# spdes/chirpgp

Hardware: AMD Instinct MI355X
Metric: filter+smoother trial-steps/s (batch x T / wall) (higher is better)
Workload: dtype f64; 1 GPU; C2: discrete EKF+EKS (demos/ekfs_mle.py model); d=4, T=10000, batch_per_gpu=1000, global_batch=1000, parallelism=trials sharded x1

## Files before the change

### chirpgp_amd/csrc/cgp_mfma4.hpp

```cpp
#pragma once
#include "cgp_coop4.hpp"

namespace cgp {


CGP_DEV double mfma4(double a, double b, double c) { return __builtin_amdgcn_mfma_f64_4x4x4f64(a, b, c, 0, 0, 0); }

constexpr int kCheckedChunks = 16;

struct Ekf4MfmaConst {
    double M0, M1, M2, M3, rho, ang;
    double Hr, Xi, Sig;
    double kc, ks, kj, kk;
    double SigHq, c0;
    double kcr, ksr, kja;
    double angm;
    double pa, pb, pA0, pB0, m1, m2;
    CGP_DEV void fold() { kcr = kc * rho; ksr = ks * rho; kja = kj * ang; angm = (kc != 0.0 || ks != 0.0) ? ang : 0.0; }
    CGP_DEV void fold_e1(int r, int q) {
        fold();
        angm = q == 0 ? ang : (q == 1 ? -ang : 0.0);
        pa = q < 2 ? rho : 0.0;
        pb = q == 0 ? -rho : (q == 1 ? rho : 0.0);
        pA0 = q == 2 ? M0 : (q == 3 ? M3 : 0.0);
        pB0 = q == 2 ? M1 : (q == 3 ? M2 : 0.0);
        m1 = r == q ? 1.0 : 0.0;
        m2 = r == (q ^ 1) ? 1.0 : 0.0;
    }
    template <bool E1> CGP_DEV void load(const HarmonicLCD<1>& model, const FilterIO& io, int64_t trial, int r, int q) {
        M0 = model.M[0]; M1 = model.M[1]; M2 = model.M[2]; M3 = model.M[3];
        rho = model.rho;
        ang = (model.dt * kTwoPi) * model.fs;
        Hr = io.H[trial * io.H_stride + r];
        Xi = io.Xi[trial * io.Xi_stride];
        Sig = lane_sigma_entry(model, r, q);
        const double mq = model.q;
        SigHq = (q == 1) ? mq : 0.0;
        c0 = mq + Xi;
        kc = ((q == 0 && r == 0) || (q == 1 && r == 1)) ? 1.0 : 0.0;
        ks = (q == 0 && r == 1) ? -1.0 : ((q == 1 && r == 0) ? 1.0 : 0.0);
        kj = (r == 2 && q == 0) ? -1.0 : ((r == 2 && q == 1) ? 1.0 : 0.0);
        kk = (q == 2) ? (r == 2 ? M0 : (r == 3 ? M1 : 0.0)) : ((q == 3) ? (r == 2 ? M2 : (r == 3 ? M3 : 0.0)) : 0.0);
        if constexpr (E1) fold_e1(r, q);
        else fold();
    }
};
struct Ekf4State {
    double P, ur, uq;
    CGP_DEV double u2() const { return dpp_f64<kQuadBcast2>(uq); }
    CGP_DEV double u2_replicated() const { return row_bcast_f64<2>(uq); }
    template <bool E1> CGP_DEV void load(const FilterIO& io, int64_t trial, int r, int q) {
        const double* __restrict__ m0p = io.m0 + trial * io.m0_stride;
        ur = E1 ? 0.0 : m0p[r]; uq = m0p[q];
        P = coop4_load_sym_entry(io.P0 + trial * io.P0_stride, r, q);
    }
};

template <int E1 = 0, bool GAPS = false>
CGP_DEV void ekf4_mfma_finish_j(const Ekf4MfmaConst& K, double y, double A, double B2, double kjd, Ekf4State& x, double& S, double& innov) {
    double J0T, f_r, f_q;
    if constexpr (E1 != 0) {
        f_q = fma(A, x.uq, B2 * dpp_f64<kQuadSwap1>(x.uq));
        J0T = fma(K.m1, A, K.m2 * B2);
        f_r = 0.0;
    } else {
        J0T = A;
        f_r = mfma4(J0T, x.ur, 0.0); f_q = mfma4(x.ur, J0T, 0.0);
    }
    const double RJT = fma(kjd, dpp_f64<kQuadSwap1>(f_q), J0T);
    double Pp, PHr, PHq;
    if constexpr (E1 != 0) {
        auto bcast1 = [](double v) { if constexpr (E1 == 2) return row_bcast_f64<1>(v); else return dpp_f64<kQuadBcast1>(v); };
        const double Q = mfma4(x.P, RJT, 0.0);
        const double Pa = bcast1(Q);
        PHq = mfma4(Pa, RJT, K.SigHq);
        Pp = mfma4(RJT, Q, K.Sig);
        PHr = bcast1(Pp);
        if constexpr (E1 == 1) {
            const double a = dpp_f64<kQuadBcast1>(RJT);
            S = mfma4(a, Pa, K.c0);
        } else {
            S = bcast1(PHq) + K.Xi;
        }
        innov = y - bcast1(f_q);
    } else {
        const double Q = mfma4(x.P, RJT, 0.0);
        Pp = mfma4(RJT, Q, K.Sig);
        PHr = mfma4(Pp, K.Hr, 0.0);
        PHq = mfma4(K.Hr, Pp, 0.0);
        S = mfma4(K.Hr, PHr, K.Xi);
        innov = y - mfma4(K.Hr, f_r, 0.0);
    }
    double rS = rcp_nr1(S), dy = innov;
    if constexpr (GAPS) {
        const bool gap = is_missing(y);
        rS = gap ? 0.0 : rS;
        dy = gap ? 0.0 : innov;
    }
    x.P = fma(-(PHr * rS), PHq, Pp);
    const double g = rS * dy;
    if constexpr (E1 == 0) x.ur = fma(PHr, g, f_r);
    x.uq = fma(PHq, g, f_q);
}
template <int E1 = 0, bool GAPS = false>
CGP_DEV void ekf4_mfma_finish(const Ekf4MfmaConst& K, double y, double c1, double s1, double dsp, Ekf4State& x, double& S, double& innov) {
    if constexpr (E1 != 0) {
        ekf4_mfma_finish_j<E1, GAPS>(K, y, fma(K.pa, c1, K.pA0), fma(K.pb, s1, K.pB0), K.kja * dsp, x, S, innov);
    } else {
        const double J0T = fma(K.kcr, c1, fma(K.ksr, s1, K.kk));
        ekf4_mfma_finish_j<E1, GAPS>(K, y, J0T, 0.0, K.kja * dsp, x, S, innov);
    }
}

template <int E1 = 0, bool GAPS = false>
CGP_DEV void ekf4_mfma_step_wide(const Ekf4MfmaConst& K, const WideRegs& W, double y, Ekf4State& x, double& S, double& innov, bool& bad) {
    double sp, dsp, s1, c1;
    bool ok1, ok2;
    softplus_pair_any(W, x.u2(), sp, dsp, ok1);
    fast_sincos_spec(W, K.ang * sp, s1, c1, ok2);
    bad = bad || !(ok1 && ok2);
    ekf4_mfma_finish<E1, GAPS>(K, y, c1, s1, dsp, x, S, innov);
}

template <int E1 = 0, bool GAPS = false>
CGP_DEV void ekf4_mfma_step_checked(const Ekf4MfmaConst& K, double y, Ekf4State& x, double& S, double& innov) {
    double sp, dsp, s1, c1;
    softplus_pair_uniform(x.u2(), sp, dsp);
    fast_sincos_uniform(K.ang * sp, s1, c1);
    ekf4_mfma_finish<E1, GAPS>(K, y, c1, s1, dsp, x, S, innov);
}

struct Ekf4Anchor {
    double th, A, B;
    template <int E1 = 0>
    CGP_DEV void set(const Ekf4MfmaConst& K, double sp, double c1, double s1) {
        th = K.angm * sp;
        if constexpr (E1 != 0) {
            A = fma(K.pa, c1, K.pA0);
            B = fma(K.pb, s1, K.pB0);
        } else {
            A = fma(K.kcr, c1, fma(K.ksr, s1, K.kk));
            B = fma(K.ksr, c1, -(K.kcr * s1));
        }
    }
};

template <int E1 = 0>
CGP_DEV void ekf4_anchor(const Ekf4MfmaConst& K, double u2, Ekf4Anchor& a) {
    double sp, dsp, s1, c1;
    softplus_pair_uniform(u2, sp, dsp);
    fast_sincos_uniform(K.ang * sp, s1, c1);
    a.template set<E1>(K, sp, c1, s1);
}

constexpr unsigned kIncrementBound = 0x3F780000u;
constexpr int kRegCommon = 0, kRegHigh = 1, kRegLow = 2, kRegAny = 3, kRegMid = 4;
struct Ekf4Verdict {
    unsigned u = 0u, umin = 0xFFFFFFFFu, d = 0u;
    int di = 0;
    bool any_bad = false;
    unsigned uabs = 0u;
    template <int REG = kRegCommon> CGP_DEV bool state_in_regime() const {
        if constexpr (REG == kRegAny) return !any_bad;
        if constexpr (REG == kRegMid) return uabs < 0x40000000u;
        if constexpr (REG == kRegLow) return umin >= 0xBFF80000u && u <= 0xC085DFFFu;
        constexpr unsigned lo = REG == kRegHigh ? 0x40140000u : 0x3FF80000u;
        return u <= 0x4085DFFFu && umin >= lo;
    }
    template <int REG = kRegCommon> CGP_DEV unsigned code() const {
        const bool state = __builtin_amdgcn_ballot_w64(!state_in_regime<REG>()) != 0;
        const bool jump = __builtin_amdgcn_ballot_w64((d & 0x7FFFFFFFu) >= kIncrementBound || ((unsigned)di & 0x7FFFFFFFu) >= kIncrementBound) != 0;
        return (state ? 1u : 0u) | (jump ? 2u : 0u);
    }
    template <int REG = kRegCommon> CGP_DEV unsigned long long uncommon() const {
        return __builtin_amdgcn_ballot_w64(!state_in_regime<REG>()) |
               __builtin_amdgcn_ballot_w64((d & 0x7FFFFFFFu) >= kIncrementBound || ((unsigned)di & 0x7FFFFFFFu) >= kIncrementBound);
    }
};
template <int E1, int REG = kRegCommon>
CGP_DEV void ekf4_mfma_step_spec1(const Ekf4MfmaConst& K, const SpecRegs& R, const SpecRegsHigh& RH, double y, Ekf4State& x, Ekf4Anchor& a,
                                  double& S, double& innov, Ekf4Verdict& verdict, const SpecRegsMid* RM = nullptr, const WideRegs* RW = nullptr) {
    const double u2 = (E1 == 2) ? x.u2_replicated() : x.u2();
    constexpr bool HIGH = REG == kRegHigh, LOW = REG == kRegLow, ANY = REG == kRegAny, MID = REG == kRegMid;
    double d, jfac;
    if constexpr (MID) {
        double ga, hj;
        softplus_mid_polys(*RM, u2, ga, hj);
        d = ga + fma(0.5 * K.angm, u2, -a.th);
        jfac = fma(u2, hj, 0.5 * K.kja);
    } else if constexpr (ANY) {
        double sp, dspf; bool ok;
        if (RW) softplus_pair_any(*RW, u2, sp, dspf, ok);
        else softplus_pair_any(u2, sp, dspf, ok);
        verdict.any_bad = verdict.any_bad || !ok;
        d = fma(K.angm, sp, -a.th);
        jfac = K.kja * dspf;
    } else {
        const double t = HIGH ? exp_neg_high(R, RH, u2) : exp_neg_lean1(R, LOW ? -u2 : u2);
        const double lin = LOW ? -a.th : fma(K.angm, u2, -a.th);
        double qa, dsp;
        if constexpr (HIGH) softplus_tail_high(RH, t, qa, dsp);
        else softplus_tail_lean(R, t, qa, dsp);
        d = fma(qa, t, lin);
        jfac = HIGH ? dsp : LOW ? (K.kja * t) * dsp : K.kja * dsp;
    }
    const double d2 = d * d;
    const double tau = d * fma(d2, R.c4, 0.5);
    const double sn = d * fma(d2, R.s3, 1.0);
    const double A1 = fma(tau, a.B, a.A);
    const double B = fma(-sn, A1, a.B);
    const double A = fma(tau, B, A1);
    const unsigned hx = (unsigned)__double2hiint(u2), hd = (unsigned)__double2hiint(d);
    if constexpr (MID) {
        const unsigned ha = hx & 0x7FFFFFFFu;
        verdict.uabs = verdict.uabs > ha ? verdict.uabs : ha;
    } else if constexpr (!ANY) {
        verdict.u = verdict.u > hx ? verdict.u : hx;
        verdict.umin = verdict.umin < hx ? verdict.umin : hx;
    }
    verdict.d = verdict.d > hd ? verdict.d : hd;
    verdict.di = verdict.di > (int)hd ? verdict.di : (int)hd;
    a.th += d; a.A = A; a.B = B;
    ekf4_mfma_finish_j<E1>(K, y, A, B, jfac, x, S, innov);
}

constexpr int kEkf4Unroll = 4;

#ifdef CGP_EKF4_KERNELS
template <bool E1>
CGP_DEV void ekf4_mfma_trial(const FilterIO& io, const ModelArgs& ma) {
    const int lane = threadIdx.x;
    const int r = lane >> 4, q = lane & 3;
    const FilterSpan span = filter_span(io, blockIdx.x);
    using Seg = SegRecord<4>;
    const int64_t trial = span.trial;

    HarmonicLCD<1> model;
    model.setup(ma.params + trial * ma.param_stride, ma.dt, ma.model_id);
    Ekf4MfmaConst K;
    K.template load<E1>(model, io, trial, r, q);
    Ekf4State x;
    x.template load<E1>(io, trial, r, q);
    const double* __restrict__ ys = io.record(trial);
    Tile4FilterOut out;
    out.init(io, trial, lane);
    const unsigned p_off = out.offP, m_off = out.offm;
    const bool nll_final = (io.flags & CGP_NLL_FINAL_ONLY) != 0;
    double* __restrict__ nll = (io.nll && !nll_final) ? io.nll + trial * io.T : nullptr;
    const bool want_nll = io.nll != nullptr;

    SpecRegs R;
    R.init(K.angm);
    SpecRegsHigh RH;
    RH.init(K.angm, K.kja);
    constexpr int kParkStride = 2;
    __shared__ double2 park[64 * kParkStride];
    __shared__ double ybuf[64 + 16];
    double cum = 0.0;
    int checked_left = 0, spec_off = 0, jump_streak = 0, spec_score = -4;
    unsigned n_high = 0, n_common = 0, n_redo = 0, n_checked = 0, n_high_left = 0, n_wide = 0, n_low = 0, n_mid = 0;
    Ekf4Anchor anchor_live;
    int anchor_age = -1;
    const int64_t Te = span.t_end;
    double ynext = (span.t_begin + lane < Te) ? ys[span.t_begin + lane] : 0.0;
    for (int64_t t0 = span.t_begin; t0 < Te; t0 += 64) {
        wave_lds_fence();
        const bool burn = t0 < span.t_out;
        const OobWindow Pw = out.P_window(burn), mw = out.m_window(burn);
        if (span.state && span.seg > 0 && t0 == span.t_out) {
            Seg::put_mean(span.state, Seg::kJunction, lane < 4, lane, x.uq);
            Seg::put_cov(span.state, Seg::kJunction, ((lane >> 2) & 3) == 0, r, q, x.P);
        }
        double ychunk = ynext;
        asm volatile("" : "+v"(ychunk));
        ynext = (t0 + 64 + lane < Te) ? ys[t0 + 64 + lane] : 0.0;
        const int nsteps = (Te - t0 < 64) ? (int)(Te - t0) : 64;
        const Ekf4State x0 = x;
        const unsigned hx0 = (unsigned)__builtin_amdgcn_readfirstlane(__double2hiint(x.u2()));
        const bool low = !nll_final && hx0 - 0xBFFC0000u <= 0xC085DFFFu - 0xBFFC0000u;
        const bool mid = !nll_final && (hx0 & 0x7FFFFFFFu) < 0x3FF80000u;
        const bool edge = !nll_final && !mid && (hx0 & 0x7FFFFFFFu) < 0x3FFC0000u;
        ybuf[lane] = ychunk;
        wave_lds_fence();
        Ekf4Anchor anchor0, anchor_end;
        const bool spec_allowed = spec_off == 0;
        if (!spec_allowed) anchor0 = anchor_live;
        else if (anchor_age < 0 || anchor_age >= 4) { ekf4_anchor<E1 ? 2 : 0>(K, x.u2(), anchor0); anchor_age = 0; }
        else anchor0 = anchor_live;
        auto chunk = [&](auto reg_c) {
            constexpr int REG = decltype(reg_c)::value;
            SpecRegsMid RM;
            if constexpr (REG == kRegMid) RM.init(K.angm, K.kja);
            WideRegs RW;
            if constexpr (REG == kRegAny) RW.init();
            Ekf4Anchor anchor = anchor0;
            Ekf4Verdict verdict;
            auto one = [&](int slot, unsigned k, double y) {
                double S, innov;
                ekf4_mfma_step_spec1<E1 ? 2 : 0, REG>(K, R, RH, y, x, anchor, S, innov, verdict, &RM, REG == kRegAny ? &RW : nullptr);
                park[(slot + k) * kParkStride] = make_double2(S, innov);
                const unsigned t = (unsigned)(t0 + slot);
                Pw.store_s(x.P, p_off + k * 128u, t * 128u);
                mw.store_s(x.uq, m_off + k * 32u, t * 32u);
            };
            int slot = 0;
            double2 ya = *reinterpret_cast<const double2*>(ybuf), yb = *reinterpret_cast<const double2*>(ybuf + 2);
            double2 yc = *reinterpret_cast<const double2*>(ybuf + 4), yd = *reinterpret_cast<const double2*>(ybuf + 6);
            for (; slot + 8 <= nsteps; slot += 8) {
                const double2 na = *reinterpret_cast<const double2*>(ybuf + slot + 8), nb = *reinterpret_cast<const double2*>(ybuf + slot + 10);
                const double2 nc = *reinterpret_cast<const double2*>(ybuf + slot + 12), nd = *reinterpret_cast<const double2*>(ybuf + slot + 14);
                one(slot, 0u, ya.x); one(slot, 1u, ya.y); one(slot, 2u, yb.x); one(slot, 3u, yb.y);
                one(slot, 4u, yc.x); one(slot, 5u, yc.y); one(slot, 6u, yd.x); one(slot, 7u, yd.y);
                ya = na; yb = nb; yc = nc; yd = nd;
            }
            for (; slot + 4 <= nsteps; slot += 4) {
                const double2 na = *reinterpret_cast<const double2*>(ybuf + slot + 4), nb = *reinterpret_cast<const double2*>(ybuf + slot + 6);
                one(slot, 0u, ya.x); one(slot, 1u, ya.y); one(slot, 2u, yb.x); one(slot, 3u, yb.y);
                ya = na; yb = nb;
            }
            for (; slot < nsteps; slot++) one(slot, 0u, readlane_f64(ychunk, slot));
            anchor_end = anchor;
            return verdict.template code<REG>();
        };
        unsigned uncommon = 1;
        const bool lean_tried = spec_allowed && (low || mid || (checked_left == 0 && !edge));
        if (lean_tried) {
            bool high = false;
            if constexpr (E1) high = !nll_final && hx0 - 0x401A0000u < 0x4085DFFFu - 0x401A0000u;
            if (low) {
                uncommon = chunk(std::integral_constant<int, kRegLow>{});
                if (uncommon == 0) n_low++;
            } else if (mid) {
                uncommon = chunk(std::integral_constant<int, kRegMid>{});
                if (uncommon == 0) n_mid++;
            } else {
                if (high) {
                    uncommon = chunk(std::integral_constant<int, kRegHigh>{});
                    if (uncommon != 0) { x = x0; n_high_left++; } else n_high++;
                }
                if (uncommon != 0) {
                    uncommon = chunk(std::integral_constant<int, kRegCommon>{});
                    if (uncommon == 0) n_common++;
                }
            }
        }
        if (uncommon != 0) {
            if (lean_tried) { x = x0; checked_left = (!(low || mid) && (uncommon & 1u)) ? kCheckedChunks : 1; n_redo++; }
            auto jumped = [&]() { jump_streak = jump_streak < 4 ? jump_streak + 1 : 4; if (spec_off < (1 << jump_streak)) spec_off = 1 << jump_streak; };
            auto failed = [&]() {
                spec_score = spec_score > -14 ? spec_score - 2 : -16;
                if (spec_score <= -8 && spec_off < 32) spec_off = 32;
                if (t0 == span.t_begin && spec_off < 8) spec_off = 8;
            };
            if (lean_tried) { failed(); if ((uncommon & 2u) != 0) jumped(); }
            if (spec_allowed && spec_off == 0) {
                uncommon = chunk(std::integral_constant<int, kRegAny>{});
                if (uncommon == 0) { if (!lean_tried) n_wide++; }
                else { failed(); if ((uncommon & 2u) != 0) jumped(); }
            }
        }
        if (uncommon == 0) {
            anchor_live = anchor_end; anchor_age++;
            if (jump_streak > 0) jump_streak--;
            if (spec_score < 8) spec_score++;
            if (checked_left > 0) checked_left--;
        } else {
            if (!spec_allowed) spec_off--;
            anchor_age = -1;
            x = x0;
            const bool redo = lean_tried;
            bool bad = false;
            WideRegs W;
            W.init();
            auto wide_one = [&](int slot, double y) {
                double S, innov;
                ekf4_mfma_step_wide<E1 ? 2 : 0>(K, W, y, x, S, innov, bad);
                park[slot * kParkStride] = make_double2(S, innov);
                const unsigned t = (unsigned)(t0 + slot);
                Pw.store_s(x.P, p_off, t * 128u);
                mw.store_s(x.uq, m_off, t * 32u);
            };
            int wslot = 0;
            for (; wslot + 4 <= nsteps; wslot += 4) {
                const double2 ya = *reinterpret_cast<const double2*>(ybuf + wslot), yb = *reinterpret_cast<const double2*>(ybuf + wslot + 2);
                wide_one(wslot, ya.x); wide_one(wslot + 1, ya.y); wide_one(wslot + 2, yb.x); wide_one(wslot + 3, yb.y);
            }
            for (; wslot < nsteps; wslot++) wide_one(wslot, readlane_f64(ychunk, wslot));
            if (__builtin_amdgcn_ballot_w64(bad) != 0) {
                x = x0;
                for (int slot = 0; slot < nsteps; slot++) {
                    double S, innov;
                    ekf4_mfma_step_checked<E1 ? 2 : 0>(K, readlane_f64(ychunk, slot), x, S, innov);
                    park[slot * kParkStride] = make_double2(S, innov);
                    const unsigned t = (unsigned)(t0 + slot);
                    Pw.store_s(x.P, p_off, t * 128u);
                    mw.store_s(x.uq, m_off, t * 32u);
                }
                if (!redo) n_checked++;
            } else if (!redo) n_wide++;
            if (checked_left > 0) checked_left--;
        }
        if (want_nll && !burn) {
            wave_lds_fence();
            const double2 si = park[(lane < nsteps ? lane : 0) * kParkStride];
            cum = nll_flush_wave(si.x, si.y, lane, nsteps, cum, nll ? nll + t0 : nullptr);
        }
    }
    if (span.state) {
        Seg::put_mean(span.state, Seg::kEnd, lane < 4, lane, x.uq);
        Seg::put_cov(span.state, Seg::kEnd, ((lane >> 2) & 3) == 0, r, q, x.P);
        Seg::put_nll(span.state, lane, cum);
    } else if (lane == 0 && io.nll && nll_final) io.nll[trial] = cum;
    if (io.counters && lane == 0) {
        atomicAdd(io.counters + 0, (unsigned long long)n_high); atomicAdd(io.counters + 1, (unsigned long long)n_common);
        atomicAdd(io.counters + 2, (unsigned long long)n_redo); atomicAdd(io.counters + 3, (unsigned long long)n_checked);
        atomicAdd(io.counters + 4, (unsigned long long)n_high_left); atomicAdd(io.counters + 5, (unsigned long long)n_wide);
        atomicAdd(io.counters + 6, (unsigned long long)n_low); atomicAdd(io.counters + 7, (unsigned long long)n_mid);
    }
}

template <bool E1>
CGP_DEV void kf4_mfma_trial(const FilterIO& io, const ModelArgs& ma) {
    const int lane = threadIdx.x;
    const int r = lane >> 4, q = lane & 3;
    const int64_t trial = blockIdx.x;
    const double* __restrict__ prm = ma.params + trial * ma.param_stride;
    const double JT = prm[q * 4 + r];
    const double Sig = prm[16 + r * 4 + q];
    const double* __restrict__ Hp = io.H + trial * io.H_stride;
    const double Hr = Hp[r];
    const double Xi = io.Xi[trial * io.Xi_stride];

    const double* __restrict__ m0p = io.m0 + trial * io.m0_stride;
    double ur = m0p[r], uq = m0p[q];
    double P = coop4_load_sym_entry(io.P0 + trial * io.P0_stride, r, q);

    const int64_t T = io.T;
    const double* __restrict__ ys = io.record(trial);
    Tile4FilterOut out;
    out.init(io, trial, lane);

    __shared__ double2 park[64];
    __shared__ double ybuf[64 + 8];
    double cum = 0.0;
    double ynext = (lane < T) ? ys[lane] : 0.0;
    for (int64_t t0 = 0; t0 < T; t0 += 64) {
        double ychunk = ynext;
        asm volatile("" : "+v"(ychunk));
        ynext = (t0 + 64 + lane < T) ? ys[t0 + 64 + lane] : 0.0;
        const int nsteps = (T - t0 < 64) ? (int)(T - t0) : 64;
        wave_lds_fence();
        auto one = [&](int slot, double y) {
            const double f_r = mfma4(JT, ur, 0.0), f_q = mfma4(ur, JT, 0.0);
            const double Q = mfma4(P, JT, 0.0);
            double Pp, PHr, PHq, S, innov;
            if constexpr (E1) {
                Pp = mfma4(JT, Q, Sig);
                PHq = mfma4(Hr, Pp, 0.0);
                PHr = dpp_f64<kQuadBcast1>(Pp);
                S = dpp_f64<kQuadBcast1>(PHq) + Xi;
                innov = y - dpp_f64<kQuadBcast1>(f_q);
            } else {
                Pp = mfma4(JT, Q, Sig);
                PHr = mfma4(Pp, Hr, 0.0);
                PHq = mfma4(Hr, Pp, 0.0);
                S = mfma4(Hr, PHr, Xi);
                innov = y - mfma4(Hr, f_r, 0.0);
            }
            const double rS = rcp_nr1(S);
            P = fma(-(PHr * rS), PHq, Pp);
            const double g = rS * innov;
            ur = fma(PHr, g, f_r);
            uq = fma(PHq, g, f_q);
            park[slot] = make_double2(S, innov);
            const unsigned t = (unsigned)(t0 + slot);
            out.wP.store_s(P, out.offP, t * 128u);
            out.wm.store_s(uq, out.offm, t * 32u);
        };
        ybuf[lane] = ychunk;
        wave_lds_fence();
        int slot = 0;
        double2 ya = *reinterpret_cast<const double2*>(ybuf), yb = *reinterpret_cast<const double2*>(ybuf + 2);
        for (; slot + 4 <= nsteps; slot += 4) {
            const double2 na = *reinterpret_cast<const double2*>(ybuf + slot + 4), nb = *reinterpret_cast<const double2*>(ybuf + slot + 6);
            one(slot, ya.x); one(slot + 1, ya.y); one(slot + 2, yb.x); one(slot + 3, yb.y);
            ya = na; yb = nb;
        }
        for (; slot < nsteps; slot++) one(slot, readlane_f64(ychunk, slot));
        if (out.want_nll) cum = out.flush_nll(park, lane, nsteps, cum, t0);
    }
    out.store_nll_total(io, trial, lane, cum);
}
__global__ void __launch_bounds__(64) kf4_mfma_kernel(FilterIO io, ModelArgs ma) {
    const int64_t trial = blockIdx.x;
    if (trial >= io.B) return;
    if (h_is_e1(io.H + trial * io.H_stride)) kf4_mfma_trial<true>(io, ma);
    else kf4_mfma_trial<false>(io, ma);
}
inline int launch_kf4_mfma(const FilterIO& io, const ModelArgs& ma, hipStream_t stream) {
    if (io.B <= 0 || io.T <= 0) return CGP_OK;
    if (!mfma4_rows_fit(io.T)) return CGP_E_UNSUPPORTED;
    hipLaunchKernelGGL(kf4_mfma_kernel, dim3((unsigned)io.B), dim3(64), 0, stream, io, ma);
    return hip_rc(hipGetLastError());
}

__global__ void __launch_bounds__(64) ekf4_mfma_kernel(FilterIO io, ModelArgs ma) {
    const int64_t trial = filter_span(io, blockIdx.x).trial;
    if (trial >= io.B) return;
    if (h_is_e1(io.H + trial * io.H_stride)) ekf4_mfma_trial<true>(io, ma);
    else ekf4_mfma_trial<false>(io, ma);
}


#endif

#ifdef CGP_EKF4_GAPS_KERNELS
template <bool E1>
CGP_DEV void ekf4_gaps_trial(const FilterIO& io, const ModelArgs& ma) {
    const int lane = threadIdx.x;
    const int r = lane >> 4, q = lane & 3;
    const int64_t trial = blockIdx.x;

    HarmonicLCD<1> model;
    model.setup(ma.params + trial * ma.param_stride, ma.dt, ma.model_id);
    Ekf4MfmaConst K;
    K.template load<E1>(model, io, trial, r, q);
    Ekf4State x;
    x.template load<E1>(io, trial, r, q);
    const int64_t T = io.T;
    const double* __restrict__ ys = io.record(trial);
    Tile4FilterOut out;
    out.init(io, trial, lane);
    const unsigned p_off = out.offP, m_off = out.offm;
    WideRegs W;
    W.init();

    __shared__ double2 park[64];
    __shared__ double ybuf[64];
    double cum = 0.0;
    unsigned n_wide = 0, n_checked = 0;
    double ynext = (lane < T) ? ys[lane] : 0.0;
    for (int64_t t0 = 0; t0 < T; t0 += 64) {
        wave_lds_fence();
        double ychunk = ynext;
        asm volatile("" : "+v"(ychunk));
        ynext = (t0 + 64 + lane < T) ? ys[t0 + 64 + lane] : 0.0;
        const int nsteps = (T - t0 < 64) ? (int)(T - t0) : 64;
        const Ekf4State x0 = x;
        ybuf[lane] = ychunk;
        wave_lds_fence();
        bool bad = false;
        auto wide_one = [&](int slot, double y) {
            double S, innov;
            ekf4_mfma_step_wide<E1 ? 2 : 0, true>(K, W, y, x, S, innov, bad);
            park[slot] = make_double2(S, innov);
            const unsigned t = (unsigned)(t0 + slot);
            out.wP.store_s(x.P, p_off, t * 128u);
            out.wm.store_s(x.uq, m_off, t * 32u);
        };
        int slot = 0;
        for (; slot + 4 <= nsteps; slot += 4) {
            const double2 ya = *reinterpret_cast<const double2*>(ybuf + slot), yb = *reinterpret_cast<const double2*>(ybuf + slot + 2);
            wide_one(slot, ya.x); wide_one(slot + 1, ya.y); wide_one(slot + 2, yb.x); wide_one(slot + 3, yb.y);
        }
        for (; slot < nsteps; slot++) wide_one(slot, readlane_f64(ychunk, slot));
        if (__builtin_amdgcn_ballot_w64(bad) != 0) {
            x = x0;
            for (int s = 0; s < nsteps; s++) {
                double S, innov;
                ekf4_mfma_step_checked<E1 ? 2 : 0, true>(K, readlane_f64(ychunk, s), x, S, innov);
                park[s] = make_double2(S, innov);
                const unsigned t = (unsigned)(t0 + s);
                out.wP.store_s(x.P, p_off, t * 128u);
                out.wm.store_s(x.uq, m_off, t * 32u);
            }
            n_checked++;
        } else n_wide++;
        if (out.want_nll) cum = out.template flush_nll<true>(park, lane, nsteps, cum, t0, ychunk);
    }
    out.store_nll_total(io, trial, lane, cum);
    if (io.counters && lane == 0) {
        atomicAdd(io.counters + 3, (unsigned long long)n_checked);
        atomicAdd(io.counters + 5, (unsigned long long)n_wide);
    }
}
__global__ void __launch_bounds__(64) ekf4_gaps_kernel(FilterIO io, ModelArgs ma) {
    if ((int64_t)blockIdx.x >= io.B) return;
    if (h_is_e1(io.H + (int64_t)blockIdx.x * io.H_stride)) ekf4_gaps_trial<true>(io, ma);
    else ekf4_gaps_trial<false>(io, ma);
}
inline int launch_ekf4_gaps(const FilterIO& io, const ModelArgs& ma, hipStream_t stream) {
    if (io.B <= 0 || io.T <= 0) return CGP_OK;
    if (!ekf4_mfma_fits(io) || io.segs > 1) return CGP_E_UNSUPPORTED;
    hipLaunchKernelGGL(ekf4_gaps_kernel, dim3((unsigned)io.B), dim3(64), 0, stream, io, ma);
    return hip_rc(hipGetLastError());
}
#endif


#ifdef CGP_EKF4_X4_KERNELS
template <int E1 = 0>
CGP_DEV void ekf4_mfma_step_checked_lane(const Ekf4MfmaConst& K, double y, Ekf4State& x, double& S, double& innov) {
    double sp, dsp, s1, c1;
    bool ok;
    softplus_pair_any(x.u2(), sp, dsp, ok);
    if (__builtin_expect(__builtin_amdgcn_ballot_w64(!ok) != 0, 0)) {
        double sp_n, dsp_n;
        softplus_pair(x.u2(), sp_n, dsp_n);
        sp = ok ? sp : sp_n;
        dsp = ok ? dsp : dsp_n;
    }
    fast_sincos(K.ang * sp, s1, c1);
    ekf4_mfma_finish<E1>(K, y, c1, s1, dsp, x, S, innov);
}
template <int E1 = 0>
CGP_DEV void ekf4_anchor_lane(const Ekf4MfmaConst& K, double u2, Ekf4Anchor& a) {
    double sp, dsp, s1, c1;
    softplus_pair_wide(u2, sp, dsp);
    fast_sincos(K.ang * sp, s1, c1);
    a.template set<E1>(K, sp, c1, s1);
}

template <bool DENSE, bool E1>
CGP_DEV void ekf4_mfma_x4_trials(const FilterIO& io, const ModelArgs& ma) {
    const int lane = threadIdx.x;
    const int r = lane >> 4, q = lane & 3, b = (lane >> 2) & 3;
    const int64_t first = (int64_t)blockIdx.x * 4;
    const int ntr = (io.B - first < 4) ? (int)(io.B - first) : 4;
    const int64_t trial = first + (b < ntr ? b : ntr - 1);

    HarmonicLCD<1> model;
    model.setup(ma.params + trial * ma.param_stride, ma.dt, ma.model_id);
    Ekf4MfmaConst K;
    K.template load<E1>(model, io, trial, r, q);
    Ekf4State x;
    x.template load<E1>(io, trial, r, q);

    const int64_t T = io.T;
    OobWindow mfs, Pfs;
    mfs.init(io.mfs ? io.mfs + first * T * 4 : nullptr, (int64_t)ntr * T * 32);
    Pfs.init(io.Pfs ? io.Pfs + first * T * 16 : nullptr, (int64_t)ntr * T * 128);
    const unsigned p_base = (unsigned)b * (unsigned)T * 128u + 8u * (4 * r + q);
    const unsigned m_base = (r == 0) ? (unsigned)b * (unsigned)T * 32u + 8u * q : kOobOffset;
    const bool nll_final = (io.flags & CGP_NLL_FINAL_ONLY) != 0;
    const bool want_nll = io.nll != nullptr;

    SpecRegs R;
    R.init<!DENSE>(K.angm);
    const SpecRegsHigh RH{};
    __shared__ double ych[4][64];
    __shared__ double2 park[4][64];
    double cum[4] = {0.0, 0.0, 0.0, 0.0};
    int checked_left = 0;
    for (int64_t t0 = 0; t0 < T; t0 += 64) {
        const int nsteps = (T - t0 < 64) ? (int)(T - t0) : 64;
        wave_lds_fence();
        CGP_UNROLL for (int bb = 0; bb < 4; bb++) {
            const int64_t tr = first + (bb < ntr ? bb : ntr - 1);
            ych[bb][lane] = (t0 + lane < T) ? io.record(tr)[t0 + lane] : 0.0;
        }
        wave_lds_fence();
        const Ekf4State x0 = x;
        unsigned long long uncommon = 0;
        if (checked_left == 0) {
            Ekf4Anchor anchor;
            ekf4_anchor_lane<E1 ? 1 : 0>(K, x.u2(), anchor);
            Ekf4Verdict verdict;
            auto one = [&](int slot) {
                double S, innov;
                ekf4_mfma_step_spec1<E1 ? 1 : 0>(K, R, RH, ych[b][slot], x, anchor, S, innov, verdict);
                park[b][slot] = make_double2(S, innov);
                const unsigned t = (unsigned)(t0 + slot);
                Pfs.store_s(x.P, p_base, t * 128u);
                mfs.store_s(x.uq, m_base, t * 32u);
            };
            int slot = 0;
            for (; slot + kEkf4Unroll <= nsteps; slot += kEkf4Unroll) {
                CGP_UNROLL for (int k = 0; k < kEkf4Unroll; k++) one(slot + k);
            }
            for (; slot < nsteps; slot++) one(slot);
            uncommon = verdict.uncommon();
        }
        const bool redo = uncommon != 0;
        if (checked_left > 0 || redo) {
            if (redo) { x = x0; checked_left = kCheckedChunks; }
            for (int slot = 0; slot < nsteps; slot++) {
                double S, innov;
                ekf4_mfma_step_checked_lane<E1 ? 1 : 0>(K, ych[b][slot], x, S, innov);
                park[b][slot] = make_double2(S, innov);
                const unsigned t = (unsigned)(t0 + slot);
                Pfs.store_s(x.P, p_base, t * 128u);
                mfs.store_s(x.uq, m_base, t * 32u);
            }
            checked_left--;
        }
        if (want_nll) {
            wave_lds_fence();
            CGP_UNROLL for (int bb = 0; bb < 4; bb++) {
                const double2 si = park[bb][lane < nsteps ? lane : 0];
                double* out = (!nll_final && bb < ntr) ? io.nll + (first + bb) * T + t0 : nullptr;
                cum[bb] = nll_flush_wave(si.x, si.y, lane, nsteps, cum[bb], out);
            }
        }
    }
    if (lane == 0 && io.nll && nll_final) {
        CGP_UNROLL for (int bb = 0; bb < 4; bb++) if (bb < ntr) io.nll[first + bb] = cum[bb];
    }
}

template <bool DENSE>
__global__ void __launch_bounds__(64) __attribute__((amdgpu_waves_per_eu(1, DENSE ? 2 : 1))) ekf4_mfma_x4_kernel(FilterIO io, ModelArgs ma) {
    const int64_t first = (int64_t)blockIdx.x * 4;
    if (first >= io.B) return;
    const int bq = (threadIdx.x >> 2) & 3;
    const int ntr0 = (io.B - first < 4) ? (int)(io.B - first) : 4;
    const bool e1 = h_is_e1(io.H + (first + (bq < ntr0 ? bq : ntr0 - 1)) * io.H_stride);
    if (__builtin_amdgcn_ballot_w64(!e1) == 0) ekf4_mfma_x4_trials<DENSE, true>(io, ma);
    else ekf4_mfma_x4_trials<DENSE, false>(io, ma);
}

inline int launch_ekf4_mfma_x4_impl(const FilterIO& io, const ModelArgs& ma, hipStream_t stream) {
    if (io.B <= 0 || io.T <= 0) return CGP_OK;
    if (!ekf4_mfma_x4_fits(io)) return CGP_E_UNSUPPORTED;
    if (io.B > 4096) hipLaunchKernelGGL(ekf4_mfma_x4_kernel<true>, dim3((unsigned)((io.B + 3) / 4)), dim3(64), 0, stream, io, ma);
    else hipLaunchKernelGGL(ekf4_mfma_x4_kernel<false>, dim3((unsigned)((io.B + 3) / 4)), dim3(64), 0, stream, io, ma);
    return hip_rc(hipGetLastError());
}
#endif

#ifdef CGP_EKF4_KERNELS
inline int launch_ekf4_mfma(const FilterIO& io, const ModelArgs& ma, hipStream_t stream) {
    if (io.B <= 0 || io.T <= 0) return CGP_OK;
    if (!ekf4_mfma_fits(io)) return CGP_E_UNSUPPORTED;
    hipLaunchKernelGGL(ekf4_mfma_kernel, dim3((unsigned)(io.B * (io.segs > 1 ? io.segs : 1))), dim3(64), 0, stream, io, ma);
    return hip_rc(hipGetLastError());
}

#endif

}
```

Before: 3.852 billion trial-steps/s.

## Add fast-path loop that chains speculative EKF chunks in the same regime

```diff
diff --git a/chirpgp_amd/csrc/cgp_mfma4.hpp b/chirpgp_amd/csrc/cgp_mfma4.hpp
--- a/chirpgp_amd/csrc/cgp_mfma4.hpp
+++ b/chirpgp_amd/csrc/cgp_mfma4.hpp
@@ -225,6 +225,7 @@
 }
 
 constexpr int kEkf4Unroll = 4;
+constexpr int kEkf4FastGroups = 4;
 
 #ifdef CGP_EKF4_KERNELS
 template <bool E1>
@@ -256,6 +257,7 @@
     constexpr int kParkStride = 2;
     __shared__ double2 park[64 * kParkStride];
     __shared__ double ybuf[64 + 16];
+    __shared__ double parkS[64], parkI[64];
     double cum = 0.0;
     int checked_left = 0, spec_off = 0, jump_streak = 0, spec_score = -4;
     unsigned n_high = 0, n_common = 0, n_redo = 0, n_checked = 0, n_high_left = 0, n_wide = 0, n_low = 0, n_mid = 0;
@@ -323,6 +325,7 @@
             return verdict.template code<REG>();
         };
         unsigned uncommon = 1;
+        int kept_reg = -1;
         const bool lean_tried = spec_allowed && (low || mid || (checked_left == 0 && !edge));
         if (lean_tried) {
             bool high = false;
@@ -336,11 +339,11 @@
             } else {
                 if (high) {
                     uncommon = chunk(std::integral_constant<int, kRegHigh>{});
-                    if (uncommon != 0) { x = x0; n_high_left++; } else n_high++;
+                    if (uncommon != 0) { x = x0; n_high_left++; } else { n_high++; kept_reg = kRegHigh; }
                 }
                 if (uncommon != 0) {
                     uncommon = chunk(std::integral_constant<int, kRegCommon>{});
-                    if (uncommon == 0) n_common++;
+                    if (uncommon == 0) { n_common++; kept_reg = kRegCommon; }
                 }
             }
         }
@@ -404,6 +407,70 @@
             wave_lds_fence();
             const double2 si = park[(lane < nsteps ? lane : 0) * kParkStride];
             cum = nll_flush_wave(si.x, si.y, lane, nsteps, cum, nll ? nll + t0 : nullptr);
+        }
+        if (kept_reg >= 0 && checked_left == 0 && spec_off == 0 && t0 >= span.t_out) {
+            auto fast_run = [&](auto reg_c) {
+                constexpr int REG = decltype(reg_c)::value;
+                for (;;) {
+                    const int64_t t1 = t0 + 64;
+                    if (t1 + 64 > Te) break;
+                    const unsigned hx1 = (unsigned)__builtin_amdgcn_readfirstlane(__double2hiint(x.u2()));
+                    const bool low1 = !nll_final && hx1 - 0xBFFC0000u <= 0xC085DFFFu - 0xBFFC0000u;
+                    const bool mid1 = !nll_final && (hx1 & 0x7FFFFFFFu) < 0x3FF80000u;
+                    const bool edge1 = !nll_final && !mid1 && (hx1 & 0x7FFFFFFFu) < 0x3FFC0000u;
+                    bool high1 = false;
+                    if constexpr (E1) high1 = !nll_final && hx1 - 0x401A0000u < 0x4085DFFFu - 0x401A0000u;
+                    if (low1 || mid1 || edge1 || high1 != (REG == kRegHigh)) break;
+                    wave_lds_fence();
+                    double ychunk = ynext;
+                    asm volatile("" : "+v"(ychunk));
+                    ynext = (t1 + 64 + lane < Te) ? ys[t1 + 64 + lane] : 0.0;
+                    const Ekf4State x1 = x;
+                    ybuf[lane] = ychunk;
+                    wave_lds_fence();
+                    const bool reanchor = anchor_age >= 4;
+                    Ekf4Anchor anchor;
+                    if (reanchor) ekf4_anchor<E1 ? 2 : 0>(K, x.u2(), anchor);
+                    else anchor = anchor_live;
+                    Ekf4Verdict verdict;
+                    auto one = [&](int slot, unsigned k, double y) {
+                        double S, innov;
+                        ekf4_mfma_step_spec1<E1 ? 2 : 0, REG>(K, R, RH, y, x, anchor, S, innov, verdict);
+                        parkS[slot + k] = S; parkI[slot + k] = innov;
+                        const unsigned t = (unsigned)(t1 + slot);
+                        out.wP.store_s(x.P, p_off + k * 128u, t * 128u);
+                        out.wm.store_s(x.uq, m_off + k * 32u, t * 32u);
+                    };
+                    double2 ya = *reinterpret_cast<const double2*>(ybuf), yb = *reinterpret_cast<const double2*>(ybuf + 2);
+                    double2 yc = *reinterpret_cast<const double2*>(ybuf + 4), yd = *reinterpret_cast<const double2*>(ybuf + 6);
+                    auto group8 = [&](int slot) {
+                        const double2 na = *reinterpret_cast<const double2*>(ybuf + slot + 8), nb = *reinterpret_cast<const double2*>(ybuf + slot + 10);
+                        const double2 nc = *reinterpret_cast<const double2*>(ybuf + slot + 12), nd = *reinterpret_cast<const double2*>(ybuf + slot + 14);
+                        one(slot, 0u, ya.x); one(slot, 1u, ya.y); one(slot, 2u, yb.x); one(slot, 3u, yb.y);
+                        one(slot, 4u, yc.x); one(slot, 5u, yc.y); one(slot, 6u, yd.x); one(slot, 7u, yd.y);
+                        ya = na; yb = nb; yc = nc; yd = nd;
+                    };
+#pragma unroll 1
+                    for (int slot = 0; slot < 64; slot += 8 * kEkf4FastGroups) {
+#pragma unroll
+                        for (int g = 0; g < kEkf4FastGroups; g++) group8(slot + 8 * g);
+                    }
+                    if (verdict.template code<REG>() != 0) { x = x1; ynext = ychunk; break; }
+                    t0 = t1;
+                    anchor_live = anchor; anchor_age = reanchor ? 1 : anchor_age + 1;
+                    if (jump_streak > 0) jump_streak--;
+                    if (spec_score < 8) spec_score++;
+                    if constexpr (REG == kRegHigh) n_high++;
+                    else n_common++;
+                    if (want_nll) {
+                        wave_lds_fence();
+                        const double2 si = make_double2(parkS[lane], parkI[lane]);
+                        cum = nll_flush_wave(si.x, si.y, lane, 64, cum, nll ? nll + t1 : nullptr);
+                    }
+                }
+            };
+            if (E1 && kept_reg == kRegHigh) { if constexpr (E1) fast_run(std::integral_constant<int, kRegHigh>{}); }
+            else fast_run(std::integral_constant<int, kRegCommon>{});
         }
     }
     if (span.state) {
```

New measurement: 4.020 billion trial-steps/s (median of 6 runs). +4.4%, better.
